# NVlabs/STEP

Measured on AMD Instinct MI355X. Metric: clips_per_sec_T32_224, higher is better.
Workload: dtype bf16; 1 GPU; C2: I3D backbone (BaseNet conv3d_1a..mixed_4f) forward, 8 x [3,32,224,224] clips per GPU, inputs resident in HBM, random-init weights; clips_per_gpu=8, T=32, HW=224, parallelism=clip-sharded replicas x1 (no data-path collective), batches_in_flight=2

## Files before the change

include/step_amd.h:

```cpp
#ifndef STEP_AMD_H
#define STEP_AMD_H

#include <stddef.h>
#include <stdint.h>

#ifdef __cplusplus
extern "C" {
#endif

#define STEP_API __attribute__((visibility("default")))

typedef void* step_stream_t;

enum { STEP_F32 = 0, STEP_BF16 = 1, STEP_F16 = 2 };
enum { STEP_NCHW = 0, STEP_NHWC = 1 };

enum {
    STEP_OK = 0,
    STEP_E_DTYPE = -1,
    STEP_E_SHAPE = -2,
    STEP_E_NULL = -3,
    STEP_E_UNSUPPORTED = -4,
    STEP_E_ALIGN = -5
};
// ... 9 lines not shown

enum {
    STEP_OPT_CONV_IMPL = 0,
    STEP_OPT_CONV_NB,
    STEP_OPT_CONV_WAVES,
    STEP_OPT_CONV_PHASED,
    STEP_OPT_CONV_GEN,
    STEP_OPT_CONV_GMODE,
    STEP_OPT_CONV_PWS,
    STEP_OPT_CONV_SPLITK,
    STEP_OPT_CONV_TAIL,
    STEP_OPT_CONV_SLOTS,
    STEP_OPT_POOL_DIRECT,
    STEP_OPT_WGRAD_MINPIX,
    STEP_OPT_WGRAD16_LDS,
    STEP_OPT_CONV_GROUP_PW,
    STEP_OPT_CLIP_VEC,
    STEP_OPT_CONV_NB_RULE,
    STEP_OPT_THROUGHPUT,
    STEP_OPT_CONV_PERSIST,
    STEP_OPT_CONV_PWS_WAVES,
    STEP_OPT_CONV_GROUP_NARROW,
    STEP_OPT_POOL_THEN_CONV,
    STEP_OPT_COUNT_
};
STEP_API int step_set_option(int option, int value);
STEP_API int step_get_option(int option, int* value);
STEP_API void step_reset_options(void);
STEP_API const char* step_option_name(int option);

STEP_API int step_roi_align_forward(const void* feat, int dtype, int layout, const float* rois, int K, int B,
                                    int C, int H, int W, int pooled_h, int pooled_w, float spatial_scale,
                                    int sampling_ratio, void* out, step_stream_t stream);

STEP_API int step_roi_align_tubes_forward(const void* feat, int dtype, const float* rois, int K, int B, int T_all, int T, int C,
                                          int H, int W, int pooled_h, int pooled_w, float spatial_scale, int sampling_ratio,
                                          void* out, step_stream_t stream);

#define STEP_ROI_BWD_GATHER 0
#define STEP_ROI_BWD_ATOMIC 1
STEP_API int step_roi_align_backward(const float* grad, int layout, const float* rois, int K, int B, int C, int H,
                                     int W, int pooled_h, int pooled_w, float spatial_scale, int sampling_ratio,
                                     int mode, float* grad_feat, step_stream_t stream);

STEP_API int step_roi_pool_forward(const void* feat, int dtype, int layout, const float* rois, int K, int B, int C,
                                   int H, int W, int pooled_h, int pooled_w, float spatial_scale, void* out,
// ... 333 lines not shown
```

step_amd/_capi.py:

```python
import ctypes as C

F32, BF16, F16 = 0, 1, 2
NCHW, NHWC = 0, 1
ROI_BWD_GATHER, ROI_BWD_ATOMIC = 0, 1
ABI_VERSION = 50

vp, fp, ip, u8p = C.c_void_p, C.c_void_p, C.c_void_p, C.c_void_p
i, f, ll, sz = C.c_int, C.c_float, C.c_longlong, C.c_size_t


class ConvDesc(C.Structure):
    _fields_ = [(n, C.c_int) for n in (
        "dtype", "N", "D", "H", "W", "Cin", "Cout", "kd", "kh", "kw", "x_cstride", "x_coff", "y_cstride", "y_coff",
        "res_cstride", "res_coff", "relu", "split", "y2_cstride", "y2_coff")]


class PackItem(C.Structure):
    _fields_ = [("w", C.c_void_p), ("perm_c", C.c_void_p), ("packed", C.c_void_p)] + [(n, C.c_int) for n in (
        "Cout", "Cin", "w_cin", "cin_lo", "kd", "kh", "kw", "dgrad", "cin_pad", "reserved")]


class ConvItem(C.Structure):
    _fields_ = [("desc", C.POINTER(ConvDesc)), ("x", C.c_void_p), ("w_packed", C.c_void_p), ("scale", C.c_void_p), ("shift", C.c_void_p),
                ("res", C.c_void_p), ("y", C.c_void_p)]
# ... 121 lines not shown
def declare(lib, strict=True):
    for name, (res, args) in SIGNATURES.items():
        if not strict and not hasattr(lib, name):
            continue
        fn = getattr(lib, name)
        fn.restype = res
        fn.argtypes = args
    return lib


_ERR = {-1: "unsupported dtype", -2: "bad shape", -3: "null pointer", -4: "unsupported configuration",
        -5: "misaligned pointer or channel count"}


def check(status, what):
    if status != 0:
        msg = _ERR.get(status, "hipError_t %d" % status) if status < 0 else "hipError_t %d" % status
        raise RuntimeError("%s failed: %s" % (what, msg))


OPTION_IDS = {name: k for k, name in enumerate((
    "conv_impl", "conv_nb", "conv_waves", "conv_phased", "conv_gen", "conv_gmode", "conv_pws", "conv_splitk", "conv_tail",
    "conv_slots", "pool_direct", "wgrad_minpix", "wgrad16_lds", "conv_group_pw", "clip_vec", "conv_nb_rule", "throughput", "conv_persist", "conv_pws_waves", "conv_group_narrow",
    "pool_then_conv"))}


def set_option(lib, name, value):
    check(lib.step_set_option(OPTION_IDS[name], int(value)), "step_set_option(%s, %r)" % (name, value))


def get_option(lib, name):
    v = C.c_int()
    check(lib.step_get_option(OPTION_IDS[name], C.byref(v)), "step_get_option(%s)" % name)
    return v.value


class options:

    def __init__(self, lib, **kw):
        self.lib, self.kw = lib, kw

    def __enter__(self):
        self.prev = {k: get_option(self.lib, k) for k in self.kw}
        for k, v in self.kw.items():
            set_option(self.lib, k, v)
        return self

# ... 5 lines not shown
```

step_amd/csrc/conv_common.h:

```cpp
#pragma once
#include "options.h"
#include "common.h"
#include <stdio.h>
#include <stdlib.h>
#include <type_traits>
#include <utility>

namespace step {


constexpr int CK = 32;

__host__ __device__ constexpr int taps_padded(int ntaps) { return (ntaps > 1 && (ntaps & 1)) ? ntaps + 1 : ntaps; }

struct ConvParams {
    const void* x; const void* w; const float* scale; const float* shift; const void* res; void* y; void* y2;
    int split, y2_cstride, y2_coff;
    int N, D, H, W, Cin, Cout;
    int x_cstride, x_coff, y_cstride, y_coff, r_cstride, r_coff;
    int relu;
    int tiles_h, tiles_w, tiles_d;
    int gtd, gth, gtw;
    int gmode;
    int gx, gy;
// ... 127 lines not shown
template <typename T>
__device__ __forceinline__ typename frag<T>::type load_b_frag(const T* p) {
    return *(const typename frag<T>::type*)p;
}

constexpr int CONV_GEN_NPIX = 768;
constexpr int CONV_GEN_NPIX_SMALL = 640;

constexpr int CONV_GEN_NPIX4 = 544;
constexpr int CONV_GEN_NPIX4_WIDE = 688;
__host__ __device__ constexpr int conv_gen_npix(int wv, int nb) {
    return wv == 8 ? (nb == 1 ? CONV_GEN_NPIX_SMALL : CONV_GEN_NPIX) : (nb >= 3 ? CONV_GEN_NPIX4 : CONV_GEN_NPIX4_WIDE);
}

constexpr int CONV_NARROW_NPIX = 1152;

static inline unsigned flat_grid(long long total, int block) {
    long long g = ceil_div64(total, block);
    if (g > 16384) g = 16384;
    return (unsigned)g;
}


struct ConvPlan { bool ok, flat, wide, deep; int impl, NB, tps, mb, wv, ph, twl, tiles_h, tiles_w, tiles_d, gtd, gth, gtw, gmode, ksplit, kchunk16, mbk, mpad, cpad; long long mtiles; };

static inline int conv_impl_override() {
    return opt(STEP_OPT_CONV_IMPL);
}

template <typename T> int conv_tap_launch(const ConvPlan& pl, const ConvParams& p, int kd, dim3 grid, step_stream_t stream);
template <typename T> int conv_tap_ph_launch(const ConvPlan& pl, const ConvParams& p, int kd, dim3 grid, step_stream_t stream);
template <> int conv_tap_ph_launch<bf16_t>(const ConvPlan& pl, const ConvParams& p, int kd, dim3 grid, step_stream_t stream);
template <> int conv_tap_ph_launch<f16_t>(const ConvPlan& pl, const ConvParams& p, int kd, dim3 grid, step_stream_t stream);
template <typename T> int conv_tap_group_launch(int twl, int NB, const ConvGroupParams& g, dim3 grid, step_stream_t stream);
template <> int conv_tap_group_launch<bf16_t>(int twl, int NB, const ConvGroupParams& g, dim3 grid, step_stream_t stream);
template <> int conv_tap_group_launch<f16_t>(int twl, int NB, const ConvGroupParams& g, dim3 grid, step_stream_t stream);
template <typename T> int conv_pw_launch(int NB, int wv, const ConvParams& p, dim3 grid, step_stream_t stream);
template <typename T> int conv_pws_launch(int nbw, const ConvParams& p, dim3 grid, step_stream_t stream);
static inline bool pws_sixteen_res(long long M, long long gx) {
    (void)M; (void)gx;
    return opt(STEP_OPT_CONV_PWS_WAVES) == 16;
}
static inline bool pws_sixteen(long long M, long long gx) {
    const int o = opt(STEP_OPT_CONV_PWS_WAVES);
    const long long g = (M + 31) >> 5;
    return o == 16 || (o == 0 && opt(STEP_OPT_THROUGHPUT) == 0 && g > gx * 8 && g <= gx * 16);
}
static inline void pws_shape(int nbw, int KC16, int& NB, int& S) {
    NB = nbw >= 3 ? 3 : nbw;
    if (nbw == 4) NB = 2;
    S = (KC16 + 3) / 4;
}
template <typename T> int conv_splitk_launch(const ConvPlan& pl, const ConvParams& p, float* ws, step_stream_t stream);

}
```

step_amd/csrc/conv_igemm.hip:

```cpp
#include "conv_common.h"

namespace step {

template <typename T, int TWL, int NB, int KD, int KH, int KW, bool FLAT, int CKT>
__global__ __launch_bounds__(256) void conv_igemm_kernel(ConvParams p) {
    constexpr int TW = 1 << TWL, TH = 128 >> TWL;
    constexpr int HH_ = TH + KH - 1, HW_ = TW + KW - 1;
    constexpr int NPIX = FLAT ? 128 : KD * HH_ * HW_;
    constexpr int ES = (int)sizeof(T);
    constexpr int VEC = 16 / ES;
    constexpr int PITCH = CKT * ES;
    constexpr int KSTEPS = CKT / 16;
    constexpr int SLOTS = PITCH / 16;
    constexpr int PPR = (16 / SLOTS) > 0 ? (16 / SLOTS) : 1;
    constexpr int NTAPS = KD * KH * KW;
    constexpr int NVEC = NPIX * SLOTS;
    constexpr int ITER = (NVEC + 255) / 256;
    typedef typename Ld16<T>::type vec16;
    typedef typename frag<T>::type frag_t;

    constexpr int LDSB = (NPIX * PITCH > 16384) ? NPIX * PITCH : 16384;
    __shared__ __attribute__((aligned(16))) unsigned char lds[LDSB];

    const int tid = threadIdx.x;
// ... 318 lines not shown
        }
    }
    return best;
}

static bool prefer_four_waves(const ConvPlan& p8, const ConvPlan& p4, const step_conv_desc* d) {
    (void)p4;
    const long long wgs8 = p8.mtiles * ceil_div(ceil_div(d->Cout, 32), 2 * p8.NB);
    return wgs8 < 64;
}

static bool prefer_four_waves_pw(const step_conv_desc* d, long long wgs8) {
    const long long M = (long long)d->N * d->D * d->H * d->W;
    return wgs8 < 128 || M >= 65536;
}

static int gen_gmode(int td, int th, int tw, int tile_px) {
    if (opt(STEP_OPT_CONV_GMODE) == 0) return 0;
    const int spr = (tw + 15) / 16;
    if ((tw & 15) < 12) return 0;
    return td * th * spr <= tile_px / 16 ? 1 : 0;
}

static ConvPlan conv_plan(const step_conv_desc* d, bool allow_pws = true, int force_waves = 0, bool no_gen = false) {
    ConvPlan pl;
    pl.ok = true; pl.wide = false; pl.tiles_h = pl.tiles_w = 0; pl.impl = 0; pl.tps = 1; pl.mb = 2; pl.wv = 8; pl.ph = 0; pl.deep = false; pl.twl = 4; pl.tiles_d = d->D; pl.gtd = pl.gth = pl.gtw = 1; pl.gmode = 0; pl.ksplit = 0; pl.kchunk16 = 0; pl.mbk = 0; pl.mpad = 0; pl.cpad = 0;
    const int nblk32 = ceil_div(d->Cout, 32);
    const bool k1 = d->kd == 1 && d->kh == 1 && d->kw == 1;
    const bool k333 = d->kd == 3 && d->kh == 3 && d->kw == 3;
    const bool k133 = d->kd == 1 && d->kh == 3 && d->kw == 3;
    pl.flat = k1;
    if (k1) {
        pl.mtiles = ceil_div64((long long)d->N * d->D * d->H * d->W, 128);
        pl.NB = pick_nb(nblk32, pl.mtiles);
        const long long mt256 = ceil_div64((long long)d->N * d->D * d->H * d->W, 256);
        const int ov1 = conv_impl_override();
        {
            const int pws_env = opt(STEP_OPT_CONV_PWS);
            const int KC16 = ceil_div(d->Cin, CK) * 2;
            const long long M = (long long)d->N * d->D * d->H * d->W;
            const bool can = d->dtype != STEP_F32 && (d->Cin % 8) == 0 && (d->x_cstride % 8) == 0 && (d->x_coff % 8) == 0 && KC16 <= 16 &&
                             (d->y_cstride % 8) == 0 && (d->y_coff % 8) == 0 && (d->Cout % 8) == 0 && (d->res_cstride % 8) == 0 && (d->res_coff % 8) == 0 &&
                             (d->split == 0 || ((d->split % 8) == 0 && (d->y2_cstride % 8) == 0 && (d->y2_coff % 8) == 0)) && M >= 1024;
            const bool wins = d->res_cstride == 0 ? (KC16 >= 12 && nblk32 >= 6 && M >= 65536) : (KC16 >= 12 && nblk32 >= 16 && M >= 49152);
            if (allow_pws && can && pws_env != 0 && (pws_env == 1 || wins) && ov1 == -1) {
                int nbmax = 152 / (ceil_div(KC16, 4) * 4);
                if (nbmax > 16) nbmax = 16;
                if (nbmax > nblk32) nbmax = nblk32;
                const int groups = ceil_div(nblk32, nbmax);
                pl.impl = 4;
                pl.NB = ceil_div(nblk32, groups);
                pl.wv = 8;
                long long gx = 256 / groups;
                if (gx < 1) gx = 1;
                const long long need = ceil_div64(ceil_div64(M, 32), 8);
                if (gx > need) gx = need;
                pl.mtiles = gx;
                return pl;
            }
        }
        if (ov1 == 5 || (ov1 != 0 && d->Cin >= 128 && d->Cout >= 64 && mt256 * ceil_div(nblk32, 2) >= 32)) {
            pl.impl = 2;
            const int waves_env = opt(STEP_OPT_CONV_WAVES);
            const long long wgs8 = mt256 * ceil_div(nblk32, 2 * pick_nb_tap(nblk32, mt256));
            const bool four = waves_env == 4 || (waves_env != 8 && prefer_four_waves_pw(d, wgs8));
            pl.wv = four ? 4 : 8;
            pl.mtiles = four ? ceil_div64((long long)d->N * d->D * d->H * d->W, 128) : mt256;
            pl.NB = pick_nb_tap(nblk32, pl.mtiles, four ? 512 : 256);
            return pl;
        }
        const bool splitk_ok = opt(STEP_OPT_CONV_SPLITK) != 0;
        const long long M = (long long)d->N * d->D * d->H * d->W;
        if (splitk_ok && ov1 != 0 && d->Cin >= 512 && (d->Cin % 8) == 0 && (M <= 1024 || (M <= 4096 && d->Cout < 64)) && pl.mtiles * nblk32 < 64) {
            pl.impl = 3;
            pl.mbk = M <= 32 ? 1 : (M <= 64 ? 2 : 4);
            const int KC16 = ceil_div(d->Cin, CK) * 2;
            const long long mt = ceil_div64(M, pl.mbk * 32);
            int ks = (int)(512 / (mt * nblk32));
            if (ks < 1) ks = 1;
            pl.kchunk16 = ceil_div(KC16, ks);
// ... 126 lines not shown
    if (!pl.ok) return STEP_E_UNSUPPORTED;
    if (p.x2 && pl.impl != 2) return STEP_E_UNSUPPORTED;
    if (p.x2 && pl.wv == 8 && pl.NB == 3) pl.NB = 2;
    if (pl.impl == 3) {
        const size_t need = (size_t)pl.ksplit * pl.mpad * pl.cpad * sizeof(float);
        if (ws && ws_bytes >= need && ((uintptr_t)ws % 16) == 0) return conv_splitk_launch<T>(pl, p, (float*)ws, stream);
        pl.impl = 0; pl.mtiles = ceil_div64(p.Mtot, 128); pl.NB = pick_nb(p.nblk32, pl.mtiles); pl.deep = d->Cin >= 256;
    }
    p.tiles_h = pl.tiles_h; p.tiles_w = pl.tiles_w; p.tiles_d = pl.tiles_d;
    p.gtd = pl.gtd; p.gth = pl.gth; p.gtw = pl.gtw; p.gmode = pl.gmode;
    conv_set_box_magic(p, d->kh, d->kw);
    auto grid1d = [&](int groups) {
        p.gx = (int)pl.mtiles; p.gy = groups;
        const long long tot = pl.mtiles * groups;
        p.gbase = 0; p.gcount = (int)((tot + 7) / 8 * 8);
        p.gpersist = 0;
        const long long slots_ = opt(STEP_OPT_CONV_SLOTS) > 0 ? opt(STEP_OPT_CONV_SLOTS) : 256;
        if (opt(STEP_OPT_CONV_PERSIST) != 0 && groups == 1 && pl.impl == 1 && pl.ph == 1 && pl.NB == 3 && p.pre_w && p.pool_row && tot > slots_)
            p.gpersist = (int)(slots_ / 8 * 8 > 0 ? slots_ / 8 * 8 : 8);
        return dim3((unsigned)p.gcount);
    };
    if (pl.impl == 4) {
        if (p.vec_epi && (!p.res || ((p.r_cstride % 8) == 0 && (p.r_coff % 8) == 0 && ((uintptr_t)p.res % 16) == 0)))
            return conv_pws_launch<T>(pl.NB, p, dim3((unsigned)pl.mtiles, (unsigned)ceil_div(p.nblk32, pl.NB)), stream);
        pl = conv_plan(d, false);
    }
    if (pl.impl == 2) {
        dim3 grid = grid1d(ceil_div(p.nblk32, 2 * pl.NB));
        return conv_pw_launch<T>(pl.NB, pl.wv, p, grid, stream);
    }
    if (pl.impl == 1) {
        const int groups = ceil_div(p.nblk32, 2 * pl.NB);
        const long long slots = opt(STEP_OPT_CONV_SLOTS) > 0 ? opt(STEP_OPT_CONV_SLOTS) : 256;
        const long long tail = pl.mtiles % slots;
        const bool tail_ok = opt(STEP_OPT_CONV_TAIL) != 0;
        const int tgroups = ceil_div(p.nblk32, 2);
        const bool box_ok = pl.twl != 0 || (pl.gtd + d->kd - 1) * (pl.gth + d->kh - 1) * (pl.gtw + d->kw - 1) <= conv_gen_npix(8, 1);
        if (tail_ok && box_ok && pl.wv == 8 && groups == 1 && pl.NB > 1 && pl.mtiles > slots && tail > 0 && tail * 4 <= slots && tail * tgroups <= slots) {
            const long long all = pl.mtiles;
            pl.mtiles = all - tail;
            dim3 grid = grid1d(1);
            int rc = conv_tap_launch<T>(pl, p, d->kd, grid, stream);
            if (rc != STEP_OK) return rc;
            ConvPlan pt = pl;
            pt.NB = 1; pt.mtiles = tail;
            p.gpersist = 0;
            p.tile0 = (int)(all - tail);
// ... 581 lines not shown
        step_conv_desc cpw;
        ConvParams ppw;
        with_pw = conv_group_pw_params(items[sel.pw], canon[0].dtype, cpw, ppw, base);
    }
    const char* t = canon[0].dtype == STEP_BF16 ? "step::bf16_t" : "step::f16_t";
    if (any_narrow)
        snprintf(buf, (size_t)buflen, "void step::conv_tap_group%s_kernel_narrow<%s, %d>(step::ConvGroupParams)", with_pw ? "_pw" : "", t, NBc);
    else
        snprintf(buf, (size_t)buflen, "void step::conv_tap_group%s_kernel<%s, %d, %d, 3, 3, 3, 2, 2, 8, 1>(step::ConvGroupParams)", with_pw ? "_pw" : "", t,
                 pls[0].twl, NBc);
    return STEP_OK;
}


int step_conv_kernel_name(const step_conv_desc* d, char* buf, int buflen) {
    if (!d || !buf || buflen <= 0) return STEP_E_NULL;
    const step_conv_desc canon = canonical_desc(d);
    d = &canon;
    const ConvPlan pl = conv_plan(d);
    if (!pl.ok) return STEP_E_UNSUPPORTED;
    const char* t = d->dtype == STEP_F32 ? "float" : (d->dtype == STEP_BF16 ? "step::bf16_t" : "step::f16_t");
    if (pl.impl == 3)
        snprintf(buf, (size_t)buflen, "void step::pw_splitk_kernel<%s, %d>(step::ConvParams, float*, int, int, int)", t, pl.mbk);
    else if (pl.impl == 4) {
        int nb, ksteps;
        pws_shape(pl.NB, ceil_div(d->Cin, CK) * 2, nb, ksteps);
        const long long M_ = (long long)d->N * d->D * d->H * d->W;
        const bool w16 = d->res_cstride == 0 && pws_sixteen(M_, pl.mtiles);
        if (d->res_cstride != 0) {
            snprintf(buf, (size_t)buflen, "void step::conv_pws_kernel<%s, %d, %d, 8, true>(step::ConvParams, int)", t, nb, ksteps);
        } else snprintf(buf, (size_t)buflen, "void step::conv_pws_kernel<%s, %d, %d, %d, false>(step::ConvParams, int)", t, w16 ? (nb > 2 ? 2 : nb) : nb, ksteps, w16 ? 16 : 8);
    }
    else if (pl.impl == 2)
        snprintf(buf, (size_t)buflen, "void step::conv_pw_kernel<%s, %d, %d>(step::ConvParams)", t, pl.NB, pl.wv);
    else if (pl.impl == 1)
        snprintf(buf, (size_t)buflen, "void step::conv_tap_kernel<%s, %d, %d, %d, %d, %d, %d, %d, %d, %d>(step::ConvParams)", t,
                 pl.twl, pl.NB, d->kd, d->kh, d->kw, pl.tps, pl.mb, pl.wv, pl.wv == 8 ? pl.ph : 0);
    else
        snprintf(buf, (size_t)buflen, "void step::conv_igemm_kernel<%s, %d, %d, %d, %d, %d, %s, %d>(step::ConvParams)", t,
                 pl.flat ? 4 : (pl.wide ? 5 : 4), pl.NB, d->kd, d->kh, d->kw, pl.flat ? "true" : "false", pl.deep ? 128 : 32);
    return STEP_OK;
}

int step_conv_plan_info(const step_conv_desc* d, int* info, int n) {
    if (!d || !info || n < 10) return STEP_E_NULL;
    const step_conv_desc canon = canonical_desc(d);
    const ConvPlan pl = conv_plan(&canon);
    if (!pl.ok) return STEP_E_UNSUPPORTED;
    info[0] = pl.impl; info[1] = pl.twl; info[2] = pl.NB; info[3] = pl.wv; info[4] = pl.ph; info[5] = pl.gtd; info[6] = pl.gth; info[7] = pl.gtw;
    info[8] = pl.gmode; info[9] = (int)(pl.mtiles > 0x7fffffff ? 0x7fffffff : pl.mtiles);
    return STEP_OK;
}

int step_conv_pre_pool_plan_info(const step_conv_desc* d, int* info, int n) {
    if (!d || !info || n < 12) return STEP_E_NULL;
// ... 28 lines not shown
```

step_amd/csrc/conv_pw.hip:

```cpp
#include "conv_common.h"
#include "conv_pw_kernel.h"

namespace step {

template <typename T, int MBK>
__global__ __launch_bounds__(256) void pw_splitk_kernel(ConvParams p, float* __restrict__ ws, int kchunk16, int mpad, int cpad) {
    typedef typename frag<T>::type frag_t;
    __shared__ float red[4][MBK * 32][33];
    const int tid = threadIdx.x, lane = tid & 63, wave = tid >> 6, khalf = lane >> 5;
    const int nb = blockIdx.x;
    const long long m0 = (long long)blockIdx.z * (MBK * 32);
    const int KC16 = p.nchunks32 * 2;
    const int ks_beg = blockIdx.y * kchunk16, ks_end = min(ks_beg + kchunk16, KC16);
    const T* xg = (const T*)p.x;
    const T* wg = (const T*)p.w + ((size_t)nb * KC16 * 64 + lane) * 8;

    const T* arow[MBK];
    bool rok[MBK];
#pragma unroll
    for (int mb = 0; mb < MBK; ++mb) {
        const long long r = m0 + mb * 32 + (lane & 31);
        rok[mb] = r < p.Mtot;
        arow[mb] = xg + (size_t)(rok[mb] ? r : 0) * p.x_cstride + p.x_coff + khalf * 8;
    }
// ... 59 lines not shown
            else ((T*)p.y)[(size_t)row * p.y_cstride + p.y_coff + co] = elem<T>::from_f32(v);
        }
        __syncthreads();
    }
}


template <typename T16>
static int splitk_forward_t(const ConvPlan& pl, const ConvParams& p, float* ws, step_stream_t stream) {
    dim3 grid((unsigned)p.nblk32, (unsigned)pl.ksplit, (unsigned)pl.mtiles);
    switch (pl.mbk) {
        case 1: STEP_LAUNCH((pw_splitk_kernel<T16, 1>), grid, dim3(256), stream, p, ws, pl.kchunk16, pl.mpad, pl.cpad); break;
        case 2: STEP_LAUNCH((pw_splitk_kernel<T16, 2>), grid, dim3(256), stream, p, ws, pl.kchunk16, pl.mpad, pl.cpad); break;
        default: STEP_LAUNCH((pw_splitk_kernel<T16, 4>), grid, dim3(256), stream, p, ws, pl.kchunk16, pl.mpad, pl.cpad); break;
    }
    const long long total = p.Mtot * p.Cout;
    STEP_LAUNCH((pw_splitk_finish_kernel<T16>), dim3(flat_grid(total, 32)), dim3(256), stream, p, (const float*)ws, pl.ksplit, pl.mpad, pl.cpad);
    return STEP_LAUNCH_CHECK();
}


constexpr int PWS_LDSW = 152 * 1024;
constexpr int PWS_WV = 8;
constexpr int PWS_MAXB = 16;

constexpr int pws_pf(int WV, int NB, int S, bool RES) {
    return WV == 16 ? ((NB == 2 && S == 4) ? 2 : 4) : (RES ? ((NB == 3 && S == 4) ? 4 : 6) : 8);
}
template <typename T, int NB, int S, int WV = PWS_WV, bool RES = false>
__global__ __launch_bounds__(WV * 64) void conv_pws_kernel(ConvParams p, int NBW) {
    constexpr bool DBUF = WV == 8;
    static_assert(sizeof(T) == 2, "16-bit storage types");
    typedef typename frag<T>::type frag_t;
    __shared__ __attribute__((aligned(16))) unsigned char lds[PWS_LDSW + 2 * PWS_MAXB * 32 * 4];
    const int tid = threadIdx.x, lane = tid & 63, khalf = lane >> 5;
#ifdef STEP_EMUL
    const int wave = tid >> 6;
#else
    const int wave = __builtin_amdgcn_readfirstlane(tid >> 6);
#endif
    const int KC16 = p.nchunks32 * 2;
    const int nbw0 = blockIdx.y * NBW;
    const int nbwv = min(NBW, p.nblk32 - nbw0);
    constexpr int KCP = 4 * S;
    {
        const u32x4* src = (const u32x4*)((const unsigned char*)p.w + (size_t)nbw0 * KC16 * 1024);
        const u32x4 z = {0u, 0u, 0u, 0u};
        for (int v = tid; v < nbwv * KCP * 64; v += WV * 64) {
            const int blk = v / (KCP * 64), rem = v % (KCP * 64), kc = rem >> 6;
            ((u32x4*)lds)[v] = kc < KC16 ? src[(blk * KC16 + kc) * 64 + (rem & 63)] : z;
        }
        float* sc = (float*)(lds + PWS_LDSW);
        for (int i = tid; i < nbwv * 32; i += WV * 64) {
            const int co = nbw0 * 32 + i;
            sc[i] = (p.scale && co < p.Cout) ? p.scale[co] : 1.f;
            sc[PWS_MAXB * 32 + i] = (p.shift && co < p.Cout) ? p.shift[co] : 0.f;
        }
    }
    __syncthreads();
    const float* scl = (const float*)(lds + PWS_LDSW);
    const float* shl = scl + PWS_MAXB * 32;
    const long long ngroups = (p.Mtot + 31) >> 5;
    const long long gstride = (long long)gridDim.x * WV;
    const T* xg = (const T*)p.x;

    frag_t xa[DBUF ? 2 : 1][S * 4];
    auto load_group = [&](auto setc, long long g) {
        constexpr int SET = DBUF ? decltype(setc)::value : 0;
        const long long gm = g * 32 + (lane & 31);
        const bool ok = g < ngroups && gm < p.Mtot;
        const T* xp = xg + (size_t)(ok ? gm : 0) * p.x_cstride + p.x_coff + 8 * khalf;
#pragma unroll
        for (int j = 0; j < S * 4; ++j) {
            frag_t v = {0, 0, 0, 0, 0, 0, 0, 0};
            if (ok && j * 16 + 8 * khalf < p.Cin) v = *(const frag_t*)(xp + j * 16);
            xa[SET][j] = v;
        }
    };
    auto group = [&](auto setc, long long g) {
        constexpr int SET = DBUF ? decltype(setc)::value : 0;
        const long long gm = g * 32 + (lane & 31);
        const bool ok = gm < p.Mtot;
        for (int b0 = 0; b0 < nbwv; b0 += NB) {
            f32x16 acc[NB];
#pragma unroll
            for (int i = 0; i < NB; ++i)
#pragma unroll
                for (int r = 0; r < 16; ++r) acc[i][r] = 0.f;
            const unsigned char* wb[NB];
#pragma unroll
            for (int i = 0; i < NB; ++i) wb[i] = lds + ((size_t)min(b0 + i, nbwv - 1) * KCP * 64 + lane) * 16;
            u32x4 rv[RES ? NB : 1][2];
            if constexpr (RES) {
                const T* rp = (const T*)p.res + (size_t)(ok ? gm : 0) * p.r_cstride + p.r_coff + nbw0 * 32 + 8 * khalf;
#pragma unroll
                for (int i = 0; i < NB; ++i)
#pragma unroll
                    for (int h = 0; h < 2; ++h) {
                        const int c8 = (b0 + i) * 32 + 16 * h;
                        u32x4 r = {0u, 0u, 0u, 0u};
                        if (ok && b0 + i < nbwv && nbw0 * 32 + c8 + 8 * khalf < p.Cout) r = *(const u32x4*)(rp + c8);
                        rv[i][h] = r;
                    }
// ... 43 lines not shown
                    d[q][1] = (unsigned)elem<T>::bits16(v[2]) | ((unsigned)elem<T>::bits16(v[3]) << 16);
                }
#pragma unroll
                for (int h = 0; h < 2; ++h) {
                    lane32_swap(d[2 * h][0], d[2 * h + 1][0]);
                    lane32_swap(d[2 * h][1], d[2 * h + 1][1]);
                    const int co = nbw0 * 32 + (b0 + i) * 32 + 16 * h + 8 * khalf;
#ifdef STEP_EXP_PWS_NOSTORE
                    if (ok && b0 + i < nbwv && co < p.Cout && d[2 * h][0] == 0x7fc17fc1u) {
#else
                    if (ok && b0 + i < nbwv && co < p.Cout) {
#endif
                        const u32x4 o = {d[2 * h][0], d[2 * h][1], d[2 * h + 1][0], d[2 * h + 1][1]};
                        if (p.split > 0 && co >= p.split) *(u32x4*)((T*)p.y2 + (size_t)gm * p.y2_cstride + p.y2_coff + (co - p.split)) = o;
                        else *(u32x4*)((T*)p.y + (size_t)gm * p.y_cstride + p.y_coff + co) = o;
                    }
                }
            }
        }
    };
    typedef std::integral_constant<int, 0> I0;
    typedef std::integral_constant<int, 1> I1;
    long long g = (long long)blockIdx.x * WV + wave;
    if (g >= ngroups) return;
    if constexpr (!DBUF) {
        for (; g < ngroups; g += gstride) {
            load_group(I0(), g);
            group(I0(), g);
        }
        return;
    }
    load_group(I0(), g);
    while (true) {
        load_group(I1(), g + gstride);
        group(I0(), g);
        g += gstride;
        if (g >= ngroups) break;
        load_group(I0(), g + gstride);
        group(I1(), g);
        g += gstride;
        if (g >= ngroups) break;
    }
}

template <typename T, int NB>
static void conv_pws_launch_s16(int S, const ConvParams& p, int nbw, dim3 grid, step_stream_t stream) {
    switch (S) {
        case 1: STEP_LAUNCH((conv_pws_kernel<T, NB, 1, 16>), grid, dim3(1024), stream, p, nbw); break;
        case 2: STEP_LAUNCH((conv_pws_kernel<T, NB, 2, 16>), grid, dim3(1024), stream, p, nbw); break;
        case 3: STEP_LAUNCH((conv_pws_kernel<T, NB, 3, 16>), grid, dim3(1024), stream, p, nbw); break;
        default: STEP_LAUNCH((conv_pws_kernel<T, NB, 4, 16>), grid, dim3(1024), stream, p, nbw); break;
    }
}
template <typename T, int NB>
static void conv_pws_launch_res(int S, const ConvParams& p, int nbw, dim3 grid, step_stream_t stream) {
    switch (S) {
        case 1: STEP_LAUNCH((conv_pws_kernel<T, NB, 1, PWS_WV, true>), grid, dim3(PWS_WV * 64), stream, p, nbw); break;
        case 2: STEP_LAUNCH((conv_pws_kernel<T, NB, 2, PWS_WV, true>), grid, dim3(PWS_WV * 64), stream, p, nbw); break;
        case 3: STEP_LAUNCH((conv_pws_kernel<T, NB, 3, PWS_WV, true>), grid, dim3(PWS_WV * 64), stream, p, nbw); break;
        default: STEP_LAUNCH((conv_pws_kernel<T, NB, 4, PWS_WV, true>), grid, dim3(PWS_WV * 64), stream, p, nbw); break;
    }
}
template <typename T, int NB>
static void conv_pws_launch_s(int S, const ConvParams& p, int nbw, dim3 grid, step_stream_t stream) {
    switch (S) {
        case 1: STEP_LAUNCH((conv_pws_kernel<T, NB, 1>), grid, dim3(PWS_WV * 64), stream, p, nbw); break;
        case 2: STEP_LAUNCH((conv_pws_kernel<T, NB, 2>), grid, dim3(PWS_WV * 64), stream, p, nbw); break;
        case 3: STEP_LAUNCH((conv_pws_kernel<T, NB, 3>), grid, dim3(PWS_WV * 64), stream, p, nbw); break;
        default: STEP_LAUNCH((conv_pws_kernel<T, NB, 4>), grid, dim3(PWS_WV * 64), stream, p, nbw); break;
    }
}
template <typename T>
int conv_pws_launch(int nbw, const ConvParams& p, dim3 grid, step_stream_t stream) {
    int NB, S;
    pws_shape(nbw, p.nchunks32 * 2, NB, S);
    if (p.res) {
        if (NB == 1) conv_pws_launch_res<T, 1>(S, p, nbw, grid, stream);
        else if (NB == 2) conv_pws_launch_res<T, 2>(S, p, nbw, grid, stream);
        else conv_pws_launch_res<T, 3>(S, p, nbw, grid, stream);
        return STEP_LAUNCH_CHECK();
    }
    if (pws_sixteen(p.Mtot, grid.x)) {
        if (NB == 1) conv_pws_launch_s16<T, 1>(S, p, nbw, grid, stream);
        else conv_pws_launch_s16<T, 2>(S, p, nbw, grid, stream);
        return STEP_LAUNCH_CHECK();
    }
    if (NB == 1) conv_pws_launch_s<T, 1>(S, p, nbw, grid, stream);
    else if (NB == 2) conv_pws_launch_s<T, 2>(S, p, nbw, grid, stream);
    else conv_pws_launch_s<T, 3>(S, p, nbw, grid, stream);
    return STEP_LAUNCH_CHECK();
}
template <>
int conv_pws_launch<float>(int, const ConvParams&, dim3, step_stream_t) { return STEP_E_UNSUPPORTED; }
template int conv_pws_launch<bf16_t>(int, const ConvParams&, dim3, step_stream_t);
template int conv_pws_launch<f16_t>(int, const ConvParams&, dim3, step_stream_t);

template <typename T>
int conv_pw_launch(int NB, int wv, const ConvParams& p, dim3 grid, step_stream_t stream) {
    if (p.x2) {
        if constexpr (sizeof(T) == 2) {
            if (wv == 4) {
                switch (NB) {
                    case 1: STEP_LAUNCH((conv_pw2_kernel<T, 1, 4>), grid, dim3(256), stream, p); break;
                    case 2: STEP_LAUNCH((conv_pw2_kernel<T, 2, 4>), grid, dim3(256), stream, p); break;
                    default: STEP_LAUNCH((conv_pw2_kernel<T, 3, 4>), grid, dim3(256), stream, p); break;
                }
                return STEP_LAUNCH_CHECK();
            }
            switch (NB) {
                case 1: STEP_LAUNCH((conv_pw2_kernel<T, 1, 8>), grid, dim3(512), stream, p); break;
                case 2: STEP_LAUNCH((conv_pw2_kernel<T, 2, 8>), grid, dim3(512), stream, p); break;
                default: return STEP_E_UNSUPPORTED;
            }
            return STEP_LAUNCH_CHECK();
        } else {
            return STEP_E_UNSUPPORTED;
        }
    }
// ... 27 lines not shown
```

step_amd/csrc/options.hip:

```cpp
#include <atomic>
#include <limits.h>

#include "options.h"

namespace step {

namespace {
struct OptSpec { const char* name; int def, lo, hi; };
constexpr OptSpec SPEC[STEP_OPT_COUNT_] = {
    {"conv_impl", -1, -1, 5},
    {"conv_nb", 0, 0, 3},
    {"conv_waves", 0, 0, 8},
    {"conv_phased", 2, 0, 2},
    {"conv_gen", 93, 0, 100},
    {"conv_gmode", 1, 0, 1},
    {"conv_pws", -1, -1, 1},
    {"conv_splitk", 1, 0, 1},
    {"conv_tail", 1, 0, 1},
    {"conv_slots", 0, 0, 1 << 20},
    {"pool_direct", 0, 0, 1},
    {"wgrad_minpix", 0, 0, 1 << 24},
    {"wgrad16_lds", 1, 0, 2},
    {"conv_group_pw", 1 << 20, 0, 1 << 20},
    {"clip_vec", 1, 0, 1},
    {"conv_nb_rule", 0, 0, 1},
    {"throughput", 0, 0, 1},
    {"conv_persist", 1, 0, 1},
    {"conv_pws_waves", 0, 0, 16},
    {"conv_group_narrow", 1, 0, 2},
    {"pool_then_conv", 1, 0, 2},
};
std::atomic<int> g_delta[STEP_OPT_COUNT_];
}

int opt(int id) { return SPEC[id].def + g_delta[id].load(std::memory_order_relaxed); }

}

using namespace step;

extern "C" {

int step_set_option(int option, int value) {
    if (option < 0 || option >= STEP_OPT_COUNT_) return STEP_E_SHAPE;
    if (value < SPEC[option].lo || value > SPEC[option].hi) return STEP_E_SHAPE;
    if (option == STEP_OPT_CONV_WAVES && value != 0 && value != 4 && value != 8) return STEP_E_SHAPE;
    if (option == STEP_OPT_CONV_PWS_WAVES && value != 0 && value != 8 && value != 16) return STEP_E_SHAPE;
    if (option == STEP_OPT_CONV_IMPL && (value == 3 || value == 4)) return STEP_E_SHAPE;
    g_delta[option].store(value - SPEC[option].def, std::memory_order_relaxed);
    return STEP_OK;
}

int step_get_option(int option, int* value) {
// ... 16 lines not shown
```

Measured before the change: 7867 clips/s.

## Stage pointwise-conv activations through swizzled per-wave LDS patches with coalesced loads

Adds a staged variant of the persistent pointwise conv kernel. Each wave loads activation rows with coalesced 16-byte row-contiguous reads into registers, writes them to a swizzled per-wave LDS patch, then reads back MFMA fragments. The first group's load is issued before weight staging to overlap with it. The staged form is selected by default only when it does not increase the number of weight groups. It reserves part of the weight LDS budget for patches and adds wave-level LDS syncs.

```diff
diff --git a/include/step_amd.h b/include/step_amd.h
--- a/include/step_amd.h
+++ b/include/step_amd.h
@@ -55,6 +55,7 @@
     STEP_OPT_CONV_PWS_WAVES,
     STEP_OPT_CONV_GROUP_NARROW,
     STEP_OPT_POOL_THEN_CONV,
+    STEP_OPT_CONV_PWS_STAGE,
     STEP_OPT_COUNT_
 };
 STEP_API int step_set_option(int option, int value);
diff --git a/step_amd/_capi.py b/step_amd/_capi.py
--- a/step_amd/_capi.py
+++ b/step_amd/_capi.py
@@ -167,7 +167,7 @@
 OPTION_IDS = {name: k for k, name in enumerate((
     "conv_impl", "conv_nb", "conv_waves", "conv_phased", "conv_gen", "conv_gmode", "conv_pws", "conv_splitk", "conv_tail",
     "conv_slots", "pool_direct", "wgrad_minpix", "wgrad16_lds", "conv_group_pw", "clip_vec", "conv_nb_rule", "throughput", "conv_persist", "conv_pws_waves", "conv_group_narrow",
-    "pool_then_conv"))}
+    "pool_then_conv", "conv_pws_stage"))}
 
 
 def set_option(lib, name, value):
diff --git a/step_amd/csrc/conv_common.h b/step_amd/csrc/conv_common.h
--- a/step_amd/csrc/conv_common.h
+++ b/step_amd/csrc/conv_common.h
@@ -173,7 +173,7 @@
 }
 
 
-struct ConvPlan { bool ok, flat, wide, deep; int impl, NB, tps, mb, wv, ph, twl, tiles_h, tiles_w, tiles_d, gtd, gth, gtw, gmode, ksplit, kchunk16, mbk, mpad, cpad; long long mtiles; };
+struct ConvPlan { bool ok, flat, wide, deep, stg; int impl, NB, tps, mb, wv, ph, twl, tiles_h, tiles_w, tiles_d, gtd, gth, gtw, gmode, ksplit, kchunk16, mbk, mpad, cpad; long long mtiles; };
 
 static inline int conv_impl_override() {
     return opt(STEP_OPT_CONV_IMPL);
@@ -187,11 +187,7 @@
 template <> int conv_tap_group_launch<bf16_t>(int twl, int NB, const ConvGroupParams& g, dim3 grid, step_stream_t stream);
 template <> int conv_tap_group_launch<f16_t>(int twl, int NB, const ConvGroupParams& g, dim3 grid, step_stream_t stream);
 template <typename T> int conv_pw_launch(int NB, int wv, const ConvParams& p, dim3 grid, step_stream_t stream);
-template <typename T> int conv_pws_launch(int nbw, const ConvParams& p, dim3 grid, step_stream_t stream);
-static inline bool pws_sixteen_res(long long M, long long gx) {
-    (void)M; (void)gx;
-    return opt(STEP_OPT_CONV_PWS_WAVES) == 16;
-}
+template <typename T> int conv_pws_launch(const ConvPlan& pl, const ConvParams& p, dim3 grid, step_stream_t stream);
 static inline bool pws_sixteen(long long M, long long gx) {
     const int o = opt(STEP_OPT_CONV_PWS_WAVES);
     const long long g = (M + 31) >> 5;
@@ -202,6 +198,19 @@
     if (nbw == 4) NB = 2;
     S = (KC16 + 3) / 4;
 }
+static inline int pws_weight_chunks(bool stg, int wv) { return 152 - (stg ? 4 * wv : 0); }
+struct PwsForm { int NB, S, wv; bool res, stg; };
+static inline PwsForm pws_form(int nbw, int KC16, int wv, bool res, bool stg) {
+    PwsForm f;
+    pws_shape(nbw, KC16, f.NB, f.S);
+    f.wv = res ? 8 : wv;
+    if (f.wv == 16 && f.NB > 2) f.NB = 2;
+    f.res = res; f.stg = stg;
+    return f;
+}
+static inline void pws_kernel_name(char* buf, int buflen, const char* t, const PwsForm& f) {
+    snprintf(buf, (size_t)buflen, "void step::conv_pws%s_kernel<%s, %d, %d, %d, %s>(step::ConvParams, int)", f.stg ? "_stg" : "", t, f.NB, f.S, f.wv, f.res ? "true" : "false");
+}
 template <typename T> int conv_splitk_launch(const ConvPlan& pl, const ConvParams& p, float* ws, step_stream_t stream);
 
 }
diff --git a/step_amd/csrc/conv_igemm.hip b/step_amd/csrc/conv_igemm.hip
--- a/step_amd/csrc/conv_igemm.hip
+++ b/step_amd/csrc/conv_igemm.hip
@@ -364,9 +364,17 @@
     return td * th * spr <= tile_px / 16 ? 1 : 0;
 }
 
+static bool pws_stage_rule(const step_conv_desc* d, int KC16, int nblk32, long long M, int wv) {
+    if (d->res_cstride != 0 || M < 65536) return false;
+    const int kcp = ceil_div(KC16, 4) * 4;
+    const int plain = pws_weight_chunks(false, wv) / kcp, staged = pws_weight_chunks(true, wv) / kcp;
+    if (staged < 1) return false;
+    return ceil_div(nblk32, plain > 16 ? 16 : plain) == ceil_div(nblk32, staged > 16 ? 16 : staged);
+}
+
 static ConvPlan conv_plan(const step_conv_desc* d, bool allow_pws = true, int force_waves = 0, bool no_gen = false) {
     ConvPlan pl;
-    pl.ok = true; pl.wide = false; pl.tiles_h = pl.tiles_w = 0; pl.impl = 0; pl.tps = 1; pl.mb = 2; pl.wv = 8; pl.ph = 0; pl.deep = false; pl.twl = 4; pl.tiles_d = d->D; pl.gtd = pl.gth = pl.gtw = 1; pl.gmode = 0; pl.ksplit = 0; pl.kchunk16 = 0; pl.mbk = 0; pl.mpad = 0; pl.cpad = 0;
+    pl.ok = true; pl.stg = false; pl.wide = false; pl.tiles_h = pl.tiles_w = 0; pl.impl = 0; pl.tps = 1; pl.mb = 2; pl.wv = 8; pl.ph = 0; pl.deep = false; pl.twl = 4; pl.tiles_d = d->D; pl.gtd = pl.gth = pl.gtw = 1; pl.gmode = 0; pl.ksplit = 0; pl.kchunk16 = 0; pl.mbk = 0; pl.mpad = 0; pl.cpad = 0;
     const int nblk32 = ceil_div(d->Cout, 32);
     const bool k1 = d->kd == 1 && d->kh == 1 && d->kw == 1;
     const bool k333 = d->kd == 3 && d->kh == 3 && d->kw == 3;
@@ -386,18 +394,30 @@
                              (d->split == 0 || ((d->split % 8) == 0 && (d->y2_cstride % 8) == 0 && (d->y2_coff % 8) == 0)) && M >= 1024;
             const bool wins = d->res_cstride == 0 ? (KC16 >= 12 && nblk32 >= 6 && M >= 65536) : (KC16 >= 12 && nblk32 >= 16 && M >= 49152);
             if (allow_pws && can && pws_env != 0 && (pws_env == 1 || wins) && ov1 == -1) {
-                int nbmax = 152 / (ceil_div(KC16, 4) * 4);
-                if (nbmax > 16) nbmax = 16;
-                if (nbmax > nblk32) nbmax = nblk32;
-                const int groups = ceil_div(nblk32, nbmax);
+                auto shape = [&](bool stg, int wv_budget) {
+                    int nbmax = pws_weight_chunks(stg, wv_budget) / (ceil_div(KC16, 4) * 4);
+                    if (nbmax > 16) nbmax = 16;
+                    if (nbmax > nblk32) nbmax = nblk32;
+                    const int groups = ceil_div(nblk32, nbmax);
+                    pl.NB = ceil_div(nblk32, groups);
+                    long long gx = 256 / groups;
+                    if (gx < 1) gx = 1;
+                    const long long need = ceil_div64(ceil_div64(M, 32), 8);
+                    if (gx > need) gx = need;
+                    pl.mtiles = gx;
+                    pl.wv = (d->res_cstride == 0 && pws_sixteen(M, gx)) ? 16 : 8;
+                    pl.stg = stg;
+                };
                 pl.impl = 4;
-                pl.NB = ceil_div(nblk32, groups);
-                pl.wv = 8;
-                long long gx = 256 / groups;
-                if (gx < 1) gx = 1;
-                const long long need = ceil_div64(ceil_div64(M, 32), 8);
-                if (gx > need) gx = need;
-                pl.mtiles = gx;
+                shape(false, 8);
+                const int stage = opt(STEP_OPT_CONV_PWS_STAGE);
+                if (stage == 2 || (stage == 1 && pws_stage_rule(d, KC16, nblk32, M, pl.wv))) {
+                    shape(true, 16);
+                    if (pl.wv != 16) {
+                        shape(true, 8);
+                        pl.wv = 8;
+                    }
+                }
                 return pl;
             }
         }
@@ -570,7 +590,7 @@
     };
     if (pl.impl == 4) {
         if (p.vec_epi && (!p.res || ((p.r_cstride % 8) == 0 && (p.r_coff % 8) == 0 && ((uintptr_t)p.res % 16) == 0)))
-            return conv_pws_launch<T>(pl.NB, p, dim3((unsigned)pl.mtiles, (unsigned)ceil_div(p.nblk32, pl.NB)), stream);
+            return conv_pws_launch<T>(pl, p, dim3((unsigned)pl.mtiles, (unsigned)ceil_div(p.nblk32, pl.NB)), stream);
         pl = conv_plan(d, false);
     }
     if (pl.impl == 2) {
@@ -1198,15 +1218,8 @@
     const char* t = d->dtype == STEP_F32 ? "float" : (d->dtype == STEP_BF16 ? "step::bf16_t" : "step::f16_t");
     if (pl.impl == 3)
         snprintf(buf, (size_t)buflen, "void step::pw_splitk_kernel<%s, %d>(step::ConvParams, float*, int, int, int)", t, pl.mbk);
-    else if (pl.impl == 4) {
-        int nb, ksteps;
-        pws_shape(pl.NB, ceil_div(d->Cin, CK) * 2, nb, ksteps);
-        const long long M_ = (long long)d->N * d->D * d->H * d->W;
-        const bool w16 = d->res_cstride == 0 && pws_sixteen(M_, pl.mtiles);
-        if (d->res_cstride != 0) {
-            snprintf(buf, (size_t)buflen, "void step::conv_pws_kernel<%s, %d, %d, 8, true>(step::ConvParams, int)", t, nb, ksteps);
-        } else snprintf(buf, (size_t)buflen, "void step::conv_pws_kernel<%s, %d, %d, %d, false>(step::ConvParams, int)", t, w16 ? (nb > 2 ? 2 : nb) : nb, ksteps, w16 ? 16 : 8);
-    }
+    else if (pl.impl == 4)
+        pws_kernel_name(buf, buflen, t, pws_form(pl.NB, ceil_div(d->Cin, CK) * 2, pl.wv, d->res_cstride != 0, pl.stg));
     else if (pl.impl == 2)
         snprintf(buf, (size_t)buflen, "void step::conv_pw_kernel<%s, %d, %d>(step::ConvParams)", t, pl.NB, pl.wv);
     else if (pl.impl == 1)
diff --git a/step_amd/csrc/conv_pw.hip b/step_amd/csrc/conv_pw.hip
--- a/step_amd/csrc/conv_pw.hip
+++ b/step_amd/csrc/conv_pw.hip
@@ -105,13 +105,26 @@
 
 constexpr int PWS_LDSW = 152 * 1024;
 constexpr int PWS_WV = 8;
+constexpr int PWS_PATCH = 4096;
 constexpr int PWS_MAXB = 16;
 
 constexpr int pws_pf(int WV, int NB, int S, bool RES) {
     return WV == 16 ? ((NB == 2 && S == 4) ? 2 : 4) : (RES ? ((NB == 3 && S == 4) ? 4 : 6) : 8);
 }
-template <typename T, int NB, int S, int WV = PWS_WV, bool RES = false>
-__global__ __launch_bounds__(WV * 64) void conv_pws_kernel(ConvParams p, int NBW) {
+__device__ __forceinline__ int pws_swz(int r) { return (r >> 1) & 7; }
+__device__ __forceinline__ void wave_lds_sync() {
+#ifdef STEP_EMUL
+    const int none = 0;
+    hipemu::exchange_begin(&none, 4);
+    hipemu::exchange_end();
+#else
+    __builtin_amdgcn_fence(__ATOMIC_RELEASE, "wavefront");
+    __builtin_amdgcn_wave_barrier();
+    __builtin_amdgcn_fence(__ATOMIC_ACQUIRE, "wavefront");
+#endif
+}
+template <typename T, int NB, int S, int WV, bool RES, bool STG>
+__device__ __forceinline__ void conv_pws_body(const ConvParams& p, int NBW) {
     constexpr bool DBUF = WV == 8;
     static_assert(sizeof(T) == 2, "16-bit storage types");
     typedef typename frag<T>::type frag_t;
@@ -126,7 +139,7 @@
     const int nbw0 = blockIdx.y * NBW;
     const int nbwv = min(NBW, p.nblk32 - nbw0);
     constexpr int KCP = 4 * S;
-    {
+    auto stage_weights = [&]() {
         const u32x4* src = (const u32x4*)((const unsigned char*)p.w + (size_t)nbw0 * KC16 * 1024);
         const u32x4 z = {0u, 0u, 0u, 0u};
         for (int v = tid; v < nbwv * KCP * 64; v += WV * 64) {
@@ -139,17 +152,47 @@
             sc[i] = (p.scale && co < p.Cout) ? p.scale[co] : 1.f;
             sc[PWS_MAXB * 32 + i] = (p.shift && co < p.Cout) ? p.shift[co] : 0.f;
         }
-    }
-    __syncthreads();
+    };
     const float* scl = (const float*)(lds + PWS_LDSW);
     const float* shl = scl + PWS_MAXB * 32;
     const long long ngroups = (p.Mtot + 31) >> 5;
     const long long gstride = (long long)gridDim.x * WV;
     const T* xg = (const T*)p.x;
 
-    frag_t xa[DBUF ? 2 : 1][S * 4];
+    frag_t xa[(DBUF && !STG) ? 2 : 1][S * 4];
+    unsigned char* const patch = lds + PWS_LDSW - (WV - wave) * PWS_PATCH;
+    const int pfrag = (lane & 31) * 128, sfrag = pws_swz(lane & 31);
+    u32x4 xr[STG ? S * 4 : 1];
+    auto load_rows = [&](long long g) {
+#pragma unroll
+        for (int i = 0; i < 4; ++i) {
+            const long long gm = g * 32 + i * 8 + (lane >> 3);
+            const bool ok = g < ngroups && gm < p.Mtot;
+            const T* xp = xg + (size_t)(ok ? gm : 0) * p.x_cstride + p.x_coff + 8 * (lane & 7);
+#pragma unroll
+            for (int s = 0; s < S; ++s) {
+                u32x4 v = {0u, 0u, 0u, 0u};
+                if (ok && s * 64 + 8 * (lane & 7) < p.Cin) v = *(const u32x4*)(xp + s * 64);
+                xr[STG ? s * 4 + i : 0] = v;
+            }
+        }
+    };
+    auto rows_to_frags = [&]() {
+#pragma unroll
+        for (int s = 0; s < S; ++s) {
+#pragma unroll
+            for (int i = 0; i < 4; ++i) {
+                const int row = i * 8 + (lane >> 3);
+                *(u32x4*)(patch + row * 128 + (((lane & 7) ^ pws_swz(row)) << 4)) = xr[STG ? s * 4 + i : 0];
+            }
+            wave_lds_sync();
+#pragma unroll
+            for (int j = 0; j < 4; ++j) xa[0][s * 4 + j] = *(const frag_t*)(patch + pfrag + (((2 * j + khalf) ^ sfrag) << 4));
+            wave_lds_sync();
+        }
+    };
     auto load_group = [&](auto setc, long long g) {
-        constexpr int SET = DBUF ? decltype(setc)::value : 0;
+        constexpr int SET = (DBUF && !STG) ? decltype(setc)::value : 0;
         const long long gm = g * 32 + (lane & 31);
         const bool ok = g < ngroups && gm < p.Mtot;
         const T* xp = xg + (size_t)(ok ? gm : 0) * p.x_cstride + p.x_coff + 8 * khalf;
@@ -161,7 +204,7 @@
         }
     };
     auto group = [&](auto setc, long long g) {
-        constexpr int SET = DBUF ? decltype(setc)::value : 0;
+        constexpr int SET = (DBUF && !STG) ? decltype(setc)::value : 0;
         const long long gm = g * 32 + (lane & 31);
         const bool ok = gm < p.Mtot;
         for (int b0 = 0; b0 < nbwv; b0 += NB) {
@@ -251,78 +294,87 @@
     typedef std::integral_constant<int, 0> I0;
     typedef std::integral_constant<int, 1> I1;
     long long g = (long long)blockIdx.x * WV + wave;
+    if constexpr (STG) load_rows(g);
+    stage_weights();
+    __syncthreads();
     if (g >= ngroups) return;
-    if constexpr (!DBUF) {
+    if constexpr (STG) {
+        while (true) {
+            rows_to_frags();
+            if constexpr (DBUF) load_rows(g + gstride);
+            group(I0(), g);
+            g += gstride;
+            if (g >= ngroups) break;
+            if constexpr (!DBUF) load_rows(g);
+        }
+    } else if constexpr (!DBUF) {
         for (; g < ngroups; g += gstride) {
             load_group(I0(), g);
             group(I0(), g);
         }
-        return;
-    }
-    load_group(I0(), g);
-    while (true) {
-        load_group(I1(), g + gstride);
-        group(I0(), g);
-        g += gstride;
-        if (g >= ngroups) break;
-        load_group(I0(), g + gstride);
-        group(I1(), g);
-        g += gstride;
-        if (g >= ngroups) break;
-    }
-}
-
-template <typename T, int NB>
-static void conv_pws_launch_s16(int S, const ConvParams& p, int nbw, dim3 grid, step_stream_t stream) {
-    switch (S) {
-        case 1: STEP_LAUNCH((conv_pws_kernel<T, NB, 1, 16>), grid, dim3(1024), stream, p, nbw); break;
-        case 2: STEP_LAUNCH((conv_pws_kernel<T, NB, 2, 16>), grid, dim3(1024), stream, p, nbw); break;
-        case 3: STEP_LAUNCH((conv_pws_kernel<T, NB, 3, 16>), grid, dim3(1024), stream, p, nbw); break;
-        default: STEP_LAUNCH((conv_pws_kernel<T, NB, 4, 16>), grid, dim3(1024), stream, p, nbw); break;
-    }
-}
-template <typename T, int NB>
-static void conv_pws_launch_res(int S, const ConvParams& p, int nbw, dim3 grid, step_stream_t stream) {
-    switch (S) {
-        case 1: STEP_LAUNCH((conv_pws_kernel<T, NB, 1, PWS_WV, true>), grid, dim3(PWS_WV * 64), stream, p, nbw); break;
-        case 2: STEP_LAUNCH((conv_pws_kernel<T, NB, 2, PWS_WV, true>), grid, dim3(PWS_WV * 64), stream, p, nbw); break;
-        case 3: STEP_LAUNCH((conv_pws_kernel<T, NB, 3, PWS_WV, true>), grid, dim3(PWS_WV * 64), stream, p, nbw); break;
-        default: STEP_LAUNCH((conv_pws_kernel<T, NB, 4, PWS_WV, true>), grid, dim3(PWS_WV * 64), stream, p, nbw); break;
-    }
-}
-template <typename T, int NB>
+    } else {
+        load_group(I0(), g);
+        while (true) {
+            load_group(I1(), g + gstride);
+            group(I0(), g);
+            g += gstride;
+            if (g >= ngroups) break;
+            load_group(I0(), g + gstride);
+            group(I1(), g);
+            g += gstride;
+            if (g >= ngroups) break;
+        }
+    }
+}
+template <typename T, int NB, int S, int WV = PWS_WV, bool RES = false>
+__global__ __launch_bounds__(WV * 64) void conv_pws_kernel(ConvParams p, int NBW) { conv_pws_body<T, NB, S, WV, RES, false>(p, NBW); }
+template <typename T, int NB, int S, int WV = PWS_WV, bool RES = false>
+__global__ __launch_bounds__(WV * 64) void conv_pws_stg_kernel(ConvParams p, int NBW) { conv_pws_body<T, NB, S, WV, RES, true>(p, NBW); }
+
+template <typename T, int NB, int WV, bool RES, bool STG>
 static void conv_pws_launch_s(int S, const ConvParams& p, int nbw, dim3 grid, step_stream_t stream) {
-    switch (S) {
-        case 1: STEP_LAUNCH((conv_pws_kernel<T, NB, 1>), grid, dim3(PWS_WV * 64), stream, p, nbw); break;
-        case 2: STEP_LAUNCH((conv_pws_kernel<T, NB, 2>), grid, dim3(PWS_WV * 64), stream, p, nbw); break;
-        case 3: STEP_LAUNCH((conv_pws_kernel<T, NB, 3>), grid, dim3(PWS_WV * 64), stream, p, nbw); break;
-        default: STEP_LAUNCH((conv_pws_kernel<T, NB, 4>), grid, dim3(PWS_WV * 64), stream, p, nbw); break;
-    }
+    if constexpr (STG) {
+        switch (S) {
+            case 1: STEP_LAUNCH((conv_pws_stg_kernel<T, NB, 1, WV, RES>), grid, dim3(WV * 64), stream, p, nbw); break;
+            case 2: STEP_LAUNCH((conv_pws_stg_kernel<T, NB, 2, WV, RES>), grid, dim3(WV * 64), stream, p, nbw); break;
+            case 3: STEP_LAUNCH((conv_pws_stg_kernel<T, NB, 3, WV, RES>), grid, dim3(WV * 64), stream, p, nbw); break;
+            default: STEP_LAUNCH((conv_pws_stg_kernel<T, NB, 4, WV, RES>), grid, dim3(WV * 64), stream, p, nbw); break;
+        }
+    } else {
+        switch (S) {
+            case 1: STEP_LAUNCH((conv_pws_kernel<T, NB, 1, WV, RES>), grid, dim3(WV * 64), stream, p, nbw); break;
+            case 2: STEP_LAUNCH((conv_pws_kernel<T, NB, 2, WV, RES>), grid, dim3(WV * 64), stream, p, nbw); break;
+            case 3: STEP_LAUNCH((conv_pws_kernel<T, NB, 3, WV, RES>), grid, dim3(WV * 64), stream, p, nbw); break;
+            default: STEP_LAUNCH((conv_pws_kernel<T, NB, 4, WV, RES>), grid, dim3(WV * 64), stream, p, nbw); break;
+        }
+    }
+}
+template <typename T, int WV, bool RES, bool STG>
+static void conv_pws_launch_nb(const PwsForm& f, const ConvParams& p, int nbw, dim3 grid, step_stream_t stream) {
+    if (f.NB == 1) conv_pws_launch_s<T, 1, WV, RES, STG>(f.S, p, nbw, grid, stream);
+    else if (f.NB == 2 || WV == 16) conv_pws_launch_s<T, 2, WV, RES, STG>(f.S, p, nbw, grid, stream);
+    else conv_pws_launch_s<T, WV == 16 ? 2 : 3, WV, RES, STG>(f.S, p, nbw, grid, stream);
 }
 template <typename T>
-int conv_pws_launch(int nbw, const ConvParams& p, dim3 grid, step_stream_t stream) {
-    int NB, S;
-    pws_shape(nbw, p.nchunks32 * 2, NB, S);
-    if (p.res) {
-        if (NB == 1) conv_pws_launch_res<T, 1>(S, p, nbw, grid, stream);
-        else if (NB == 2) conv_pws_launch_res<T, 2>(S, p, nbw, grid, stream);
-        else conv_pws_launch_res<T, 3>(S, p, nbw, grid, stream);
-        return STEP_LAUNCH_CHECK();
-    }
-    if (pws_sixteen(p.Mtot, grid.x)) {
-        if (NB == 1) conv_pws_launch_s16<T, 1>(S, p, nbw, grid, stream);
-        else conv_pws_launch_s16<T, 2>(S, p, nbw, grid, stream);
-        return STEP_LAUNCH_CHECK();
-    }
-    if (NB == 1) conv_pws_launch_s<T, 1>(S, p, nbw, grid, stream);
-    else if (NB == 2) conv_pws_launch_s<T, 2>(S, p, nbw, grid, stream);
-    else conv_pws_launch_s<T, 3>(S, p, nbw, grid, stream);
+int conv_pws_launch(const ConvPlan& pl, const ConvParams& p, dim3 grid, step_stream_t stream) {
+    const PwsForm f = pws_form(pl.NB, p.nchunks32 * 2, pl.wv, p.res != nullptr, pl.stg);
+    if (pl.NB * 4 * f.S > pws_weight_chunks(f.stg, f.wv)) return STEP_E_UNSUPPORTED;
+    if (f.res) {
+        if (f.stg) conv_pws_launch_nb<T, 8, true, true>(f, p, pl.NB, grid, stream);
+        else conv_pws_launch_nb<T, 8, true, false>(f, p, pl.NB, grid, stream);
+    } else if (f.wv == 16) {
+        if (f.stg) conv_pws_launch_nb<T, 16, false, true>(f, p, pl.NB, grid, stream);
+        else conv_pws_launch_nb<T, 16, false, false>(f, p, pl.NB, grid, stream);
+    } else {
+        if (f.stg) conv_pws_launch_nb<T, 8, false, true>(f, p, pl.NB, grid, stream);
+        else conv_pws_launch_nb<T, 8, false, false>(f, p, pl.NB, grid, stream);
+    }
     return STEP_LAUNCH_CHECK();
 }
 template <>
-int conv_pws_launch<float>(int, const ConvParams&, dim3, step_stream_t) { return STEP_E_UNSUPPORTED; }
-template int conv_pws_launch<bf16_t>(int, const ConvParams&, dim3, step_stream_t);
-template int conv_pws_launch<f16_t>(int, const ConvParams&, dim3, step_stream_t);
+int conv_pws_launch<float>(const ConvPlan&, const ConvParams&, dim3, step_stream_t) { return STEP_E_UNSUPPORTED; }
+template int conv_pws_launch<bf16_t>(const ConvPlan&, const ConvParams&, dim3, step_stream_t);
+template int conv_pws_launch<f16_t>(const ConvPlan&, const ConvParams&, dim3, step_stream_t);
 
 template <typename T>
 int conv_pw_launch(int NB, int wv, const ConvParams& p, dim3 grid, step_stream_t stream) {
diff --git a/step_amd/csrc/options.hip b/step_amd/csrc/options.hip
--- a/step_amd/csrc/options.hip
+++ b/step_amd/csrc/options.hip
@@ -29,6 +29,7 @@
     {"conv_pws_waves", 0, 0, 16},
     {"conv_group_narrow", 1, 0, 2},
     {"pool_then_conv", 1, 0, 2},
+    {"conv_pws_stage", 1, 0, 2},
 };
 std::atomic<int> g_delta[STEP_OPT_COUNT_];
 }
```

After: 7874 clips/s (median of 6 runs). No clear change (+0.1%).
